# privacy-scaling-explorations/zkevm-specs

Hardware: AMD Instinct MI355X
Metric: BN254 constraint-rows/sec (higher is better)
Workload: dtype u256 (BN254 Fr: 4xu64 canonical cells, u32-limb Montgomery); 1 GPU; EVM circuit, 2^18 execution steps per GPU, mixed-opcode synthetic trace (BASELINE configs[2]); RW table 816377 rows, bytecode table 43913 rows; steps_per_gpu=262144, rw_rows=816377, bytecode_rows=43913, witness_copies=3

## Files before the change

### zkevm_specs_amd/csrc/zkevm_hip.hip

```cpp
#include <hip/hip_runtime.h>
#include <hip/hip_ext.h>
#include <stddef.h>
#include <stdio.h>
#include <string.h>
#include <stdlib.h>
#include <chrono>
#include <string>
#include <vector>

#include <atomic>
#include <mutex>
#include <dlfcn.h>

#include "../../include/zkevm_hip.h"
#include "kernels.hpp"
#include "dist_tally.hpp"
#include "host_index.hpp"
#include "code_dir_build.hpp"

#define ZK_MAX_DEVICES 64
static std::mutex g_dev_mutex;
static hipStream_t g_own_stream[ZK_MAX_DEVICES] = {nullptr};
static hipStream_t g_batch_stream[ZK_MAX_DEVICES][2] = {{nullptr}};
static hipStream_t g_side_stream[ZK_MAX_DEVICES] = {nullptr};
// ... 169 lines not shown
    __shared__ u32 local[EVM_N_BINS];
    if (vblock == 0) {
        if (threadIdx.x == 0 && defer_count) *defer_count = 0u;
        if (threadIdx.x == 0) {
            tally->fail_count = 0ull;
            tally->first_fail = ~0ull;
        }
        for (u32 k = threadIdx.x; k < EVM_N_BINS; k += blockDim.x) taken[k] = 0;
    }
    for (u32 k = threadIdx.x; k < EVM_N_BINS; k += blockDim.x) local[k] = 0;
    __syncthreads();
    u32 i = vblock * blockDim.x + threadIdx.x;
    if (i < n_pairs) {
        const u32 bin = evm_state_bin((u32)steps[((u64)i * STEP_NCELLS + S_STATE) * 4]);
        bin16[i] = (uint16_t)bin;
        atomicAdd(&local[bin], 1u);
    }
    __syncthreads();
    for (u32 k = threadIdx.x; k < EVM_N_BINS; k += blockDim.x)
        if (local[k]) atomicAdd(&hist[k], local[k]);
}
__global__ void evm_state_hist_kernel(const u64* steps, u32 n_pairs, u32* hist, u32* taken, uint16_t* bin16, ZkTally* tally, u32* defer_count) {
    evm_state_hist_body(blockIdx.x, steps, n_pairs, hist, taken, bin16, tally, defer_count);
}
__device__ __forceinline__ void evm_state_scatter_body(u32 vblock, const uint16_t* bin16, u32 n_pairs, const u32* hist, u32* hist_next,
                                                       u32* taken, u32* group_start, u32* perm, u32* early_host = nullptr, u32 early_seq = 0u) {
    __shared__ u32 sa[EVM_N_BINS], sb[EVM_N_BINS];
    __shared__ u32 local[EVM_N_BINS];
    __shared__ u32 base[EVM_N_BINS];
    __shared__ u32 gsh[EVM_N_GROUPS + 1];
    const u32 k = threadIdx.x;
    u32 c = 0, c_real = 0;
    if (k < EVM_N_BINS) {
        c_real = hist[k];
        c = k < (u32)EVM_GROUP_WARM * 128u ? ((c_real + 63u) & ~63u) : c_real;
        sa[k] = c;
        local[k] = 0;
        if (vblock == 0) hist_next[k] = 0;
    }
    __syncthreads();
    u32* src = sa;
    u32* dst = sb;
    for (u32 off = 1; off < EVM_N_BINS; off <<= 1) {
        if (k < EVM_N_BINS) dst[k] = src[k] + (k >= off ? src[k - off] : 0u);
        __syncthreads();
        u32* t = src; src = dst; dst = t;
    }
    u32 excl = 0;
    if (k < EVM_N_BINS) {
        excl = src[k] - c;
        if (vblock == 0) {
            if ((k & 127u) == 0) group_start[k >> 7] = gsh[k >> 7] = excl;
            if (k == EVM_N_BINS - 1) group_start[EVM_N_GROUPS] = gsh[EVM_N_GROUPS] = src[k];
            for (u32 j = c_real; j < c; j++) perm[excl + j] = EVM_NO_PAIR;
        }
    }
    const u32 i = vblock * blockDim.x + threadIdx.x;
    u32 bin = 0, rank = 0;
    if (i < n_pairs) {
        bin = bin16[i];
        rank = atomicAdd(&local[bin], 1u);
    }
    __syncthreads();
    if (vblock == 0 && k == 0 && early_host) {
        __hip_atomic_store(&early_host[EVM_EARLY_WORD], gsh[EVM_GROUP_WARM + 1] - gsh[EVM_GROUP_WARM], __ATOMIC_RELAXED, __HIP_MEMORY_SCOPE_SYSTEM);
        __hip_atomic_store(&early_host[EVM_EARLY_WORD + 1], gsh[EVM_GROUP_COLD + 1] - gsh[EVM_GROUP_COLD], __ATOMIC_RELAXED, __HIP_MEMORY_SCOPE_SYSTEM);
        __threadfence_system();
        __hip_atomic_store(&early_host[EVM_EARLY_WORD + 2], early_seq, __ATOMIC_RELEASE, __HIP_MEMORY_SCOPE_SYSTEM);
    }
    if (k < EVM_N_BINS && local[k]) base[k] = excl + atomicAdd(&taken[k], local[k]);
    __syncthreads();
    if (i < n_pairs) perm[base[bin] + rank] = i;
}
__global__ __launch_bounds__(1024) void evm_state_scatter_kernel(const uint16_t* bin16, u32 n_pairs, const u32* hist, u32* hist_next,
                                                                 u32* taken, u32* group_start, u32* perm) {
    evm_state_scatter_body(blockIdx.x, bin16, n_pairs, hist, hist_next, taken, group_start, perm);
}
__global__ __launch_bounds__(256) void evm_open_fill_kernel(uint4* ff, u64 n_ff, uint4* zero, u64 n_zero) {
    const u64 stride = (u64)gridDim.x * blockDim.x;
    const uint4 F = make_uint4(~0u, ~0u, ~0u, ~0u), Z = make_uint4(0u, 0u, 0u, 0u);
    for (u64 i = (u64)blockIdx.x * blockDim.x + threadIdx.x; i < n_ff; i += stride) ff[i] = F;
    for (u64 i = (u64)blockIdx.x * blockDim.x + threadIdx.x; i < n_zero; i += stride) zero[i] = Z;
}
__device__ __forceinline__ void rw_prepare_quad(const ZkTable& t, u64* keys, EvmDyn* dyn, u32 vthread) {
    const u32 r = vthread >> 2, q = vthread & 3u;
    const bool in = r < t.n;
    uint4 c0 = make_uint4(0, 0, 0, 0), c1 = c0, c2 = c0;
    u64 base = 0;
    u32 flags = 3u;
    if (in) {
        const uint4* p = reinterpret_cast<const uint4*>(t.cells + (u64)r * RW_NCELLS * 4) + q;
        c0 = p[0];
        c1 = p[4];
        c2 = p[8];
        if (q == 0) {
            base = t.cells[0];
            if (t.flags) flags = t.flags[r];
        }
    }
    bool fit, dense_ok;
    u64 w0 = 0, w1 = 0, w2 = 0, w3 = 0;
    const bool z0hi = (c0.y | c0.z | c0.w) == 0u, z1hi = (c1.y | c1.z | c1.w) == 0u, z2hi = (c2.y | c2.z | c2.w) == 0u;
    const bool z0 = z0hi && c0.x == 0u, z1 = z1hi && c1.x == 0u, z2 = z2hi && c2.x == 0u;
    if (q == 0) {
        const u64 rwc = (u64)c0.x | ((u64)c0.y << 32);
        dense_ok = (c0.z | c0.w) == 0u && rwc == base + r && base + r >= base;
        fit = z1hi && c1.x <= 255u;
        w0 = (u64)(c1.x & 0xffu) << 8 | ((u64)(flags & 3u) << 56) | (1ull << 63);
        w2 = (u64)c2.x | ((u64)c2.y << 32);
        w3 = (u64)c2.z | ((u64)c2.w << 32);
    } else if (q == 1) {
        dense_ok = z0;
        fit = z1 && z2hi;
        w0 = (u64)c2.x << 24;
    } else if (q == 2) {
        dense_ok = true;
        fit = z0hi && c0.x <= 255u && (c1.z | c1.w) == 0u && z2hi && c2.x <= 255u;
        w0 = (u64)(c0.x & 0xffu) | ((u64)(c2.x & 0xffu) << 16);
        w1 = (u64)c1.x | ((u64)c1.y << 32);
    } else {
        dense_ok = true;
        fit = z0 && z1 && z2;
    }
    const u32 qshift = threadIdx.x & 60u;
    const bool fits = ((__ballot(fit) >> qshift) & 0xfull) == 0xfull;
    const unsigned long long nd = __ballot(in && !dense_ok);
    if (nd != 0ull && (threadIdx.x & 63u) == 0) atomicOr(&dyn->rw_sparse, 1u);
    if (r == 0 && q == 0 && in) dyn->rw_base = base;
#pragma unroll
    for (int m = 1; m <= 2; m <<= 1) {
        w0 |= __shfl_xor(w0, m);
        w1 |= __shfl_xor(w1, m);
        w2 |= __shfl_xor(w2, m);
        w3 |= __shfl_xor(w3, m);
    }
    if (!fits) w0 = w1 = w2 = w3 = 0;
    if (in && q < 2) {
        const u64 a = q == 0 ? w0 : w2, b2 = q == 0 ? w1 : w3;
        reinterpret_cast<uint4*>(keys + (u64)r * 4)[q] = make_uint4((u32)a, (u32)(a >> 32), (u32)b2, (u32)(b2 >> 32));
    }
}
#define EVM_OPEN_TABLES 8
struct EvmOpenTables {
    ZkTable t[EVM_OPEN_TABLES];
    u32 block_start[EVM_OPEN_TABLES + 2];
    const u64* wds;
    u32 n_wds;
    EvmDyn* dyn;
    ZkTally* tally;
    ZkTable rw;
    u64* rw_keys;
    u32 dir_block0, rw_block0;
    DirBuild dir;
    const u64* steps;
    u32 n_steps;
    u32* step_recs;
    u32 rec_block0;
    EvmSortArgs sort;
    u32 hist_block0;
    u32 lat_period;
#ifdef ZK_DIAG_P1
    u32 diag_skip;
#endif
};
__device__ __forceinline__ void evm_open_small_tables(const EvmOpenTables& o, u32 block) {
    int k = 0;
#pragma unroll
    for (int j = 1; j <= EVM_OPEN_TABLES; j++) k += block >= o.block_start[j] ? 1 : 0;
    const u32 r = (block - o.block_start[k]) * blockDim.x + threadIdx.x;
    if (k == EVM_OPEN_TABLES) {
        const bool nz = r < o.n_wds && !fr_is_zero(fr_load(o.wds + ((u64)r * 4 + 3) * 4));
        const unsigned long long b = __ballot(nz);
        if (b && (threadIdx.x & 63u) == 0) atomicAdd(&o.dyn->agg_total_wds, (u32)__popcll(b));
        return;
    }
    const ZkTable& t = o.t[k];
    const bool in = r < t.n;
    if (k == 0) {
        bool caller = false, present = false, invalid = false, bad = false;
        if (in) {
            const Fr tag = zk_table_cell(t, r, 1), lo = zk_table_cell(t, r, 3), hi = zk_table_cell(t, r, 4);
            caller = fr_eq_u64(tag, 4);
            present = caller && !(fr_is_zero(lo) && fr_is_zero(hi));
            const bool inv_row = fr_eq_u64(tag, 10);
            bad = inv_row && t.flags && (t.flags[r] & 1u);
            invalid = inv_row && fr_eq_u64(lo, 1);
        }
        const unsigned long long bc = __ballot(caller), bp = __ballot(present), bi = __ballot(invalid), bb = __ballot(bad);
        if ((threadIdx.x & 63u) == 0) {
            if (bc) atomicAdd(&o.dyn->agg_max_txs, (u32)__popcll(bc));
            if (bp) atomicAdd(&o.dyn->agg_total_txs, (u32)__popcll(bp));
            if (bi) atomicAdd(&o.dyn->agg_invalid_txs, (u32)__popcll(bi));
            if (bb) atomicOr(&o.dyn->agg_bad_invalid_rows, 1u);
        }
    }
    if (!in) return;
    u64 h;
    switch (k) {
    case 0: h = tx_key_hash(t, r); break;
    case 1: h = blk_key_hash(t, r); break;
    case 2: h = bc_key_hash(t, r); break;
    case 3: h = copy_key_hash(t, r); break;
    case 4: h = keccak_key_hash(t, r); break;
    case 5: h = expt_key_hash(t, r); break;
    case 6: h = sig_key_hash(t, r); break;
    default: h = ecc_key_hash(t, r); break;
    }
    u32* slots = const_cast<u32*>(t.slots);
    u32 s = (u32)h & t.mask;
    while (atomicCAS(&slots[s], ZK_EMPTY_SLOT, r) != ZK_EMPTY_SLOT) s = (s + 1) & t.mask;
}
__global__ __launch_bounds__(256) void evm_open_phase1_kernel(EvmOpenTables o) {
    if (blockIdx.x == 0 && threadIdx.x < 2) {
        o.tally[threadIdx.x].fail_count = 0ull;
        o.tally[threadIdx.x].first_fail = ~0ull;
    }
    u32 b = blockIdx.x;
    if (o.lat_period > 1u && b < o.rec_block0) {
        const u32 q = b / o.lat_period;
        b = (b == q * o.lat_period && q < o.rw_block0) ? q : o.rw_block0 + b - (q + 1u < o.rw_block0 ? q + 1u : o.rw_block0);
    }
#ifdef ZK_DIAG_P1
    {
        const u32 range = b < o.dir_block0 ? 1u : b < o.hist_block0 ? 2u : b < o.rw_block0 ? 4u : b < o.rec_block0 ? 8u : 16u;
        if (o.diag_skip & range) return;
    }
#endif
    if (b < o.dir_block0) evm_open_small_tables(o, b);
    else if (b < o.hist_block0) dirb_events_row(o.dir, (b - o.dir_block0) * blockDim.x + threadIdx.x);
    else if (b < o.rw_block0) evm_state_hist_body(b - o.hist_block0, o.sort.steps, o.sort.n_pairs, o.sort.hist, o.sort.taken, o.sort.bin16, o.sort.tally, o.sort.defer_count);
    else if (b < o.rec_block0) rw_prepare_quad(o.rw, o.rw_keys, o.dyn, (b - o.rw_block0) * blockDim.x + threadIdx.x);
    else evm_step_record_quad(o.steps, o.n_steps, o.step_recs, (b - o.rec_block0) * blockDim.x + threadIdx.x);
}
#define EVM_OPEN_RW_GENERIC_BLOCKS 64u
#define EVM_OPEN_P2_BLOCK 1024u
__global__ __launch_bounds__(1024) void evm_open_phase2_kernel(EvmOpenTables o, u32 scatter_blocks, u32 dir_blocks, u32 force_generic) {
    if (blockIdx.x < scatter_blocks) {
        evm_state_scatter_body(blockIdx.x, o.sort.bin16, o.sort.n_pairs, o.sort.hist, o.sort.hist_next, o.sort.taken, o.sort.group_start, o.sort.perm,
                               o.sort.early_host, o.sort.early_seq);
        return;
    }
    const u32 b = blockIdx.x - scatter_blocks;
    if (b < dir_blocks) {
        dirb_finalize_entry(o.dir, b * blockDim.x + threadIdx.x);
        return;
    }
    if (!force_generic && o.dyn->rw_sparse == 0u) return;
    if (force_generic && b == dir_blocks && threadIdx.x == 0) o.dyn->rw_sparse = 1u;
    u32* slots = const_cast<u32*>(o.rw.slots);
    const u32 stride = (gridDim.x - scatter_blocks - dir_blocks) * blockDim.x;
    for (u32 r = (b - dir_blocks) * blockDim.x + threadIdx.x; r < o.rw.n; r += stride) {
        u32 s = (u32)rw_key_hash(o.rw, r) & o.rw.mask;
        bool dup = false;
        for (;;) {
            const u32 q = atomicCAS(&slots[s], ZK_EMPTY_SLOT, r);
            if (q == ZK_EMPTY_SLOT) break;
            if (!dup && q < o.rw.n) {
                bool same = true;
                for (int c = 0; c < RW_NCELLS && same; c++) same = fr_eq(zk_table_cell(o.rw, q, c), zk_table_cell(o.rw, r, c));
                dup = same;
            }
            s = (s + 1) & o.rw.mask;
        }
        if (dup) atomicAdd(&o.dyn->agg_rw_dups, 1u);
    }
}

__global__ void fr_op_kernel(int op, const u64* a, const u64* b, u64* out, u64 n) {
    u64 i = (u64)blockIdx.x * blockDim.x + threadIdx.x;
    if (i >= n) return;
    Fr x = fr_load(a + 4 * i), y = fr_load(b + 4 * i), r;
    switch (op) {
    case 0: r = fr_add(x, y); break;
    case 1: r = fr_sub(x, y); break;
    case 2: r = fr_mul(x, y); break;
    case 3: r = fr_mont(x, y); break;
    case 4: r = fr_neg(x); break;
    case 5: r = fr_inv(x); break;
    case 6: r = fr_div(x, y); break;
    case 16: r = sp_mul_p(x, y); break;
    case 17: r = sp_sqr_p(x); break;
    case 18: r = ecc_fq_mul_hook(x, y); break;
    case 26: r = sp_sqrt_p(x); break;
    case 27: r = sp_inv_p(x); break;
    default: r = fr_zero();
    }
    for (int k = 0; k < 4; k++) out[4 * i + k] = (u64)r.v[2 * k] | ((u64)r.v[2 * k + 1] << 32);
}

__global__ __launch_bounds__(64) void evm_publish_kernel(const u32* d, u32* h, u32 seq) {
    const u32 i = threadIdx.x;
    if (i < 32u) __hip_atomic_store(&h[i], d[i], __ATOMIC_RELAXED, __HIP_MEMORY_SCOPE_SYSTEM);
    __threadfence_system();
    if (i == 0u) __hip_atomic_store(&h[32], seq, __ATOMIC_RELEASE, __HIP_MEMORY_SCOPE_SYSTEM);
}
struct EvmResultBlock {
    EvmDyn dyn;
    u32 n_deferred_twin;
    u32 pad0[(64 - sizeof(EvmDyn)) / 4 - 1];
    ZkTally tally[2];
    u32 group_start[EVM_N_GROUPS + 1];
    u32 pad1[8 - (EVM_N_GROUPS + 1)];
};
static_assert(sizeof(EvmDyn) <= 64 && sizeof(EvmResultBlock) == 128, "EvmResultBlock layout");
enum SessionKind { SESSION_BCC = 22, SESSION_SGA = 21, SESSION_ECC_ASSIGN = 20, SESSION_ECC = 19, SESSION_PIA = 18, SESSION_EXA = 17, SESSION_TXA = 16, SESSION_WITHDRAWAL = 15, SESSION_REKEY = 14, SESSION_PICOPY = 13, SESSION_PI = 12, SESSION_CPA = 11, SESSION_STATE = 1, SESSION_EVM = 2, SESSION_BYTECODE = 3, SESSION_EXP = 4, SESSION_COPY = 5, SESSION_SIGN = 6, SESSION_KECCAK = 7, SESSION_ASSIGN = 8, SESSION_ECDSA = 9, SESSION_BCA = 10 };

struct zk_session {
    SessionKind kind;
    int device = t_device;
    hipStream_t stream = t_stream;
    u64 n = 0;
    u64 eval_lo = 0, eval_hi = 0;
    bool eval_empty = false;
    std::vector<void*> owned;
    std::vector<int> owned_class;
    ZkTally* d_tally = nullptr;
    u32* d_status = nullptr;
    bool status_external = false;
    std::vector<hipEvent_t> ev;
    u32 launches = 0;
    u32 tally_pass = 0;
    ZkTally* tally_last = nullptr;
    StateArgs state;
    EvmArgs evm;
    BytecodeArgs bytecode;
    ExpArgs exp;
    CopyArgs copy;
    SignArgs sign;
    KeccakGenArgs keccak_gen;
    AssignArgs assign;
    EcdsaArgs ecdsa;
    BcaArgs bca;
    CpaArgs cpa;
// ... 272 lines not shown
    {
        DevArena& A = g_arena[s->device];
        std::lock_guard<std::mutex> lock(A.m);
        for (hipEvent_t e : s->ev) A.events.push_back(e);
        if (s->ev_open0) A.events.push_back(s->ev_open0);
        if (s->ev_open1) A.events.push_back(s->ev_open1);
        if (s->ev_fork) A.events.push_back(s->ev_fork);
        if (s->ev_join) A.events.push_back(s->ev_join);
        if (s->h_result) A.pinned.push_back(s->h_result);
    }
    delete s;
    return 0;
}

extern "C" int zk_state_open(const uint64_t* rows, const uint32_t* flags, uint64_t n, const uint64_t* mpt,
                             uint64_t n_mpt, uint32_t opts, zk_session** out) {
    ARG_TRY(t_device >= 0, "zk_state_open: call zk_init first");
    HIP_TRY(hipSetDevice(t_device));
    ARG_TRY(out && rows && n > 0 && n < (1ull << 32), "zk_state_open: bad arguments");
    ARG_TRY(n_mpt < (1ull << 31), "zk_state_open: MPT table too large");
    const bool dev = opts & ZK_OPT_DEVICE_PTRS;
    const bool compact = opts & ZK_OPT_STATE_COMPACT;
    zk_session* s = new zk_session();
    s->kind = SESSION_STATE;
    s->n = n;
    int rc = 0;
    const void* p = nullptr;
    if ((rc = stage(s, rows, (size_t)n * (compact ? 15 : ST_NCELLS) * 32, dev, &p))) goto fail;
    s->state.rows.cells = (const u64*)p;
    s->state.rows.skip = compact ? 42u : 0u;
    if ((rc = stage(s, flags, (size_t)n * 4, dev, &p))) goto fail;
    s->state.rows.flags = (const u32*)p;
    s->state.rows.n = n;
    s->state.eval_lo = 0;
    s->state.eval_hi = n;
    if ((rc = stage(s, mpt, (size_t)n_mpt * MPT_NCELLS * 32, dev, &p))) goto fail;
    s->state.mpt.cells = (const u64*)p;
    s->state.mpt.flags = nullptr;
    s->state.mpt.n = (u32)n_mpt;
    s->state.mpt.ncells = MPT_NCELLS;
    if ((rc = build_index<state_mpt_key_hash>(s, s->state.mpt, true))) goto fail;
    if ((rc = session_common_init(s))) goto fail;
    *out = s;
    return 0;
fail:
    zk_close(s);
    return rc;
}

static int table_stage(zk_session* s, ZkTable& t, const uint64_t* cells, const uint32_t* flags, uint64_t n,
                       u32 ncells, bool dev) {
    const void* p = nullptr;
    int rc;
    if ((rc = stage(s, cells, (size_t)n * ncells * 32, dev, &p))) return rc;
    t.cells = (const u64*)p;
    if ((rc = stage(s, flags, (size_t)n * 4, dev, &p))) return rc;
    t.flags = (n && flags) ? (const u32*)p : nullptr;
    t.n = (u32)n;
    t.ncells = ncells;
    return 0;
}

#ifndef ZK_HIST_BLOCK
#define ZK_HIST_BLOCK 1024
#endif
static int evm_build_perm(zk_session* s) {
    const u32 n = s->evm.n_pairs;
    u32* h_cur = (s->evm_pass & 1u) ? s->d_hist2 : s->d_hist;
    u32* h_next = (s->evm_pass & 1u) ? s->d_hist : s->d_hist2;
    s->evm_pass++;
    hipLaunchKernelGGL(evm_state_hist_kernel, dim3((n + ZK_HIST_BLOCK - 1) / ZK_HIST_BLOCK), dim3(ZK_HIST_BLOCK), 0, s->stream, s->evm.steps, n, h_cur, s->d_cursor, s->d_bin16, s->d_tally, s->evm.defer_count);
    hipLaunchKernelGGL(evm_state_scatter_kernel, dim3((n + 1023) / 1024), dim3(1024), 0, s->stream, s->d_bin16, n, h_cur, h_next, s->d_cursor,
                       s->d_group_start, s->d_perm);
    HIP_TRY(hipGetLastError());
    return 0;
}

static inline u32 index_cap(u64 n) {
    u32 cap = 16;
    while (cap < 2 * n + 2) cap <<= 1;
    return cap;
}

extern "C" int zk_evm_open(const zk_evm_tables* t, uint32_t opts, zk_session** out) {
    ARG_TRY(t_device >= 0, "zk_evm_open: call zk_init first");
    HIP_TRY(hipSetDevice(t_device));
    ARG_TRY(t && out && t->steps && t->n_steps >= 2 && t->n_steps < (1ull << 32), "zk_evm_open: bad arguments");
    ARG_TRY(t->n_rw < (1ull << 31) && t->n_bytecode < (1ull << 31) && t->n_tx < (1ull << 31) && t->n_block < (1ull << 31) &&
            t->n_copy < (1ull << 31) && t->n_keccak < (1ull << 31) && t->n_exp < (1ull << 31) && t->n_withdrawals < (1ull << 31) &&
            t->n_sig < (1ull << 31) && t->n_ecc < (1ull << 31),
            "zk_evm_open: table too large");
    ARG_TRY(t->aux_cells == 0 || (t->aux_cells >= 2 && t->aux_cells <= 64), "zk_evm_open: aux_cells must be 0 (= 2) or 2..64");
    const bool dev = opts & ZK_OPT_DEVICE_PTRS;
    const bool generic = opts & ZK_OPT_GENERIC_INDEX;
    zk_session* s = new zk_session();
    s->kind = SESSION_EVM;
    s->n = t->n_steps - 1;
    s->side_stream = (opts & ZK_OPT_SIDE_STREAM) != 0;
    int rc = 0;
    const void* p = nullptr;
    EvmArgs& E = s->evm;
    if ((rc = stage(s, t->steps, (size_t)t->n_steps * STEP_NCELLS * 32, dev, &p))) goto fail;
    E.steps = (const u64*)p;
    E.n_steps = t->n_steps;
    E.n_pairs = (u32)(t->n_steps - 1);
    if ((rc = table_stage(s, E.rw, t->rw, t->rw_flags, t->n_rw, RW_NCELLS, dev))) goto fail;
    if ((rc = table_stage(s, E.bytecode, t->bytecode, nullptr, t->n_bytecode, BYTECODE_NCELLS, dev))) goto fail;
    if ((rc = table_stage(s, E.tx, t->tx, t->tx_flags, t->n_tx, TX_NCELLS, dev))) goto fail;
    if ((rc = table_stage(s, E.block, t->block, t->block_flags, t->n_block, BLOCK_NCELLS, dev))) goto fail;
    if ((rc = table_stage(s, E.copy, t->copy, nullptr, t->n_copy, COPY_T_NCELLS, dev))) goto fail;
    if ((rc = table_stage(s, E.keccak, t->keccak, nullptr, t->n_keccak, KECCAK_NCELLS, dev))) goto fail;
    if ((rc = table_stage(s, E.exp, t->exp, nullptr, t->n_exp, EXP_T_NCELLS, dev))) goto fail;
    if ((rc = table_stage(s, E.sig, t->sig, nullptr, t->n_sig, SIG_T_NCELLS, dev))) goto fail;
    if ((rc = table_stage(s, E.ecc, t->ecc, nullptr, t->n_ecc, ECC_T_NCELLS, dev))) goto fail;
    if ((rc = table_stage(s, E.withdrawals, t->withdrawals, nullptr, t->n_withdrawals, 4, dev))) goto fail;
    E.withdrawals.slots = nullptr;
    E.withdrawals.mask = 0;
    E.aux = nullptr;
    E.aux_kind = nullptr;
    E.aux_cells = t->aux_cells ? t->aux_cells : 2u;
    if (t->aux && t->aux_kind) {
        if ((rc = stage(s, t->aux, (size_t)t->n_steps * E.aux_cells * 32, dev, &p))) goto fail;
        E.aux = (const u64*)p;
        if ((rc = stage(s, t->aux_kind, (size_t)t->n_steps * 4, dev, &p))) goto fail;
        E.aux_kind = (const u32*)p;
    }
    {
        ZkTable* const small[EVM_OPEN_TABLES] = {&E.tx, &E.block, &E.bytecode, &E.copy, &E.keccak, &E.exp, &E.sig, &E.ecc};
        const bool want_dir = !generic && t->n_bytecode != 0;
        size_t n_ff = 0;
        u32 caps[EVM_OPEN_TABLES];
        for (int k = 0; k < EVM_OPEN_TABLES; k++) { caps[k] = index_cap(small[k]->n); n_ff += caps[k]; }
        const u32 cap_rw = index_cap(E.rw.n), cap_big = want_dir ? index_cap(t->n_bytecode) : 0u;
        n_ff += (size_t)cap_rw + 2 * (size_t)cap_big + (want_dir ? DIRB_SMALL_SLOTS : 0u);
        u32* ff = nullptr;
        if ((rc = dev_alloc(s, (void**)&ff, n_ff * sizeof(u32)))) goto fail;
        u32* cur = ff;
        for (int k = 0; k < EVM_OPEN_TABLES; k++) { small[k]->slots = cur; small[k]->mask = caps[k] - 1; cur += caps[k]; }
        E.rw.slots = cur; E.rw.mask = cap_rw - 1; cur += cap_rw;
        u32* const dir_rep = cur; cur += cap_big;
        u32* const dir_first = cur; cur += cap_big;
        u32* const small_slots = cur;
        const size_t dyn_bytes = 256, hist_bytes = EVM_N_BINS * sizeof(u32), status_bytes = (((size_t)s->n * sizeof(u32)) + 15) & ~(size_t)15;
        const size_t zero_bytes = dyn_bytes + 2 * hist_bytes + status_bytes + 3 * (size_t)cap_big * 4;
        char* zero = nullptr;
        if ((rc = dev_alloc(s, (void**)&zero, zero_bytes))) goto fail;
        EvmResultBlock* const rb = (EvmResultBlock*)zero;
        EvmDyn* dyn = &rb->dyn;
        s->d_result = rb;
        if ((rc = arena_pinned(s->device, &s->h_result))) goto fail;
        {
            void* hd = nullptr;
            if (hipHostGetDevicePointer(&hd, s->h_result, 0) == hipSuccess) s->h_result_dev = (u32*)hd;
            (void)hipGetLastError();
        }
        static_assert(sizeof(EvmResultBlock) <= 256, "the result block outgrew its slot");
        static_assert((EVM_N_BINS * sizeof(u32)) % 16 == 0, "zero region pieces are 16-byte multiples");
        s->d_hist = (u32*)(zero + dyn_bytes);
        s->d_hist2 = (u32*)(zero + dyn_bytes + hist_bytes);
        s->d_status = (u32*)(zero + dyn_bytes + 2 * hist_bytes);
        u32* const dir_last = (u32*)(zero + dyn_bytes + 2 * hist_bytes + status_bytes);
        E.dyn = dyn;
        E.defer_count = &dyn->n_deferred;
        if ((rc = dev_alloc(s, (void**)&E.defer_list, (size_t)E.n_pairs * sizeof(u32)))) goto fail;
        s->d_tally = rb->tally;
        s->tally_last = s->d_tally;
        {
            const u64 n16 = n_ff / 4 + zero_bytes / 16;
            const u32 fill_grid = (u32)(n16 / 256 < 2048 ? (n16 + 255) / 256 : 2048);
            if (arena_event(s->device, &s->ev_open0) || arena_event(s->device, &s->ev_open1)) s->ev_open0 = s->ev_open1 = nullptr;
            hipExtLaunchKernelGGL(evm_open_fill_kernel, dim3(fill_grid ? fill_grid : 1u), dim3(256), 0, s->stream, s->ev_open0, nullptr, 0, (uint4*)ff,
                                  (u64)(n_ff / 4), (uint4*)zero, (u64)(zero_bytes / 16));
        }
        E.rw_dense = 0;
        E.rw_base = 0;
        E.rw_keys = nullptr;
        E.codes.n = 0;
        E.codes.mask = 0;
        E.codes.packed = nullptr;
        E.codes.entries = nullptr;
        E.codes.slots = nullptr;
        E.agg_max_txs = E.agg_total_txs = E.agg_invalid_txs = E.agg_bad_invalid_rows = E.agg_total_wds = E.agg_rw_dups = 0;
        EvmOpenTables o;
        memset(&o, 0, sizeof o);
        u32 blk = 0;
        for (int k = 0; k < EVM_OPEN_TABLES; k++) { o.t[k] = *small[k]; o.block_start[k] = blk; blk += (small[k]->n + 255u) / 256u; }
        o.block_start[EVM_OPEN_TABLES] = blk;
        blk += (u32)((t->n_withdrawals + 255) / 256);
        o.block_start[EVM_OPEN_TABLES + 1] = blk;
        o.wds = E.withdrawals.cells;
        o.n_wds = (u32)t->n_withdrawals;
        o.dyn = dyn;
        o.tally = s->d_tally;
        o.rw = E.rw;
        if (t->n_rw && !generic) {
            u64* d_keys = nullptr;
            if ((rc = dev_alloc(s, (void**)&d_keys, (size_t)t->n_rw * 32))) goto fail;
            E.rw_keys = d_keys;
            o.rw_keys = d_keys;
        }
        const u32 rw_row_blocks = o.rw_keys ? (u32)((t->n_rw + 63) / 64) : 0u;
        o.dir_block0 = blk;
        u32 dir_row_blocks = 0;
        if (want_dir) {
            DirBuild& d = o.dir;
            d.rows = E.bytecode.cells;
            d.n = (u32)t->n_bytecode;
            d.rep = dir_rep;
            d.first = dir_first;
            d.last = dir_last;
            d.runs = dir_last + cap_big;
            d.bad = dir_last + 2 * (size_t)cap_big;
            d.big_mask = cap_big - 1;
            d.small_slots = small_slots;
            d.dyn = dyn;
            if ((rc = dev_alloc(s, (void**)&d.packed, (size_t)d.n * sizeof(uint16_t)))) goto fail;
            if ((rc = dev_alloc(s, (void**)&d.entries, (size_t)DIRB_MAX_ENTRIES * sizeof(ZkCodeEntry)))) goto fail;
            if ((rc = dev_alloc(s, (void**)&d.list, (size_t)DIRB_MAX_ENTRIES * 4))) goto fail;
            dir_row_blocks = (d.n + 255u) / 256u;
            E.codes.entries = d.entries;
            E.codes.slots = d.small_slots;
            E.codes.packed = d.packed;
        }
        if ((rc = dev_alloc(s, (void**)&s->d_cursor, EVM_N_BINS * sizeof(u32)))) goto fail;
        if ((rc = dev_alloc(s, (void**)&s->d_bin16, (size_t)E.n_pairs * sizeof(uint16_t)))) goto fail;
        s->d_group_start = rb->group_start;
        if ((rc = dev_alloc(s, (void**)&s->d_perm, ((size_t)E.n_pairs + EVM_PERM_PAD + 2 * EVM_HOT_BLOCK) * sizeof(u32)))) goto fail;
        const bool sorted = !(opts & ZK_OPT_NO_STATE_SORT);
        o.hist_block0 = o.dir_block0 + dir_row_blocks;
        u32 hist_blocks = 0, scatter_blocks = 0;
        if (sorted) {
            o.sort.steps = E.steps; o.sort.n_pairs = E.n_pairs; o.sort.hist = s->d_hist; o.sort.hist_next = s->d_hist2;
            o.sort.taken = s->d_cursor; o.sort.bin16 = s->d_bin16; o.sort.group_start = s->d_group_start; o.sort.perm = s->d_perm;
            o.sort.tally = s->d_tally;
            o.sort.defer_count = E.defer_count;
            if ((opts & ZK_OPT_SINGLE_PASS) && s->h_result_dev && evm_lazy_tail_enabled() && !(opts & ZK_OPT_SIDE_STREAM)) {
                static std::atomic<u32> g_early_seq{0};
                u32 q = ++g_early_seq;
                if (!q) q = ++g_early_seq;
                __atomic_store_n(&((u32*)s->h_result)[EVM_EARLY_WORD + 2], 0u, __ATOMIC_RELEASE);
                s->early_seq = q;
                o.sort.early_host = s->h_result_dev;
                o.sort.early_seq = q;
            }
            hist_blocks = (E.n_pairs + 255u) / 256u;
            scatter_blocks = (E.n_pairs + EVM_OPEN_P2_BLOCK - 1u) / EVM_OPEN_P2_BLOCK;
            s->evm_pass = 1;
            s->perm_ready = true;
        }
        o.rw_block0 = o.hist_block0 + hist_blocks;
        o.rec_block0 = o.rw_block0 + rw_row_blocks;
        u32 rec_blocks = 0;
        E.step_recs = nullptr;
        if (!(opts & ZK_OPT_SINGLE_PASS)) {
            u32* recs = nullptr;
            if ((rc = dev_alloc(s, (void**)&recs, (size_t)t->n_steps * EVM_REC_WORDS * sizeof(u32)))) goto fail;
            o.steps = E.steps; o.n_steps = (u32)t->n_steps; o.step_recs = recs;
            E.step_recs = recs;
            rec_blocks = (u32)((t->n_steps + 63) / 64);
        }
        const u32 grid1 = o.rec_block0 + rec_blocks;
        {
            static const u32 spread = [] { const char* e = getenv("ZK_P1_LAT_SPREAD"); const int v = e ? atoi(e) : 2; return (u32)(v < 0 ? 0 : v); }();
            o.lat_period = (o.rw_block0 && spread) ? o.rec_block0 / (spread * o.rw_block0) : 0u;
        }
#ifdef ZK_DIAG_P1
        if (const char* e = getenv("ZK_DIAG_P1_SKIP")) o.diag_skip = (u32)atoi(e);
#endif
        {
            const u32 dir_blocks = want_dir ? DIRB_MAX_ENTRIES / EVM_OPEN_P2_BLOCK : 0u;
            const u32 rw_blocks = t->n_rw ? EVM_OPEN_RW_GENERIC_BLOCKS : 0u;
            bool phase2 = scatter_blocks + dir_blocks + rw_blocks != 0;
#ifdef ZK_DIAG_P1
            if (o.diag_skip) phase2 = false;
#endif
            hipExtLaunchKernelGGL(evm_open_phase1_kernel, dim3(grid1 ? grid1 : 1u), dim3(256), 0, s->stream, nullptr, phase2 ? nullptr : s->ev_open1, 0, o);
            if (phase2)
                hipExtLaunchKernelGGL(evm_open_phase2_kernel, dim3(scatter_blocks + dir_blocks + rw_blocks), dim3(EVM_OPEN_P2_BLOCK), 0, s->stream, nullptr,
                                      s->ev_open1, 0, o, scatter_blocks, dir_blocks, generic ? 1u : 0u);
        }
        if (hipGetLastError() != hipSuccess) { rc = -2; g_err = "zk_evm_open: a build kernel failed to launch"; goto fail; }
    }
    E.opts = (t->begin_with_first_step ? 1u : 0u) | (t->end_with_last_step ? 2u : 0u);
    E.prof = nullptr;
    if (getenv("ZK_EVM_PROF")) {
        if ((rc = dev_alloc(s, (void**)&E.prof, 1024 * 4 * 8 * sizeof(unsigned long long)))) goto fail;
        if (hipMemsetAsync(E.prof, 0, 1024 * 4 * 8 * sizeof(unsigned long long), s->stream) != hipSuccess) { rc = -2; goto fail; }
    }
    E.perm = (opts & ZK_OPT_NO_STATE_SORT) ? nullptr : s->d_perm;
    *out = s;
    return 0;
fail:
    zk_close(s);
    return rc;
}

static void session_timing(zk_session* s, double pass_ms, double* open_ms, double* span_ms);
static int evm_enqueue_tail(zk_session* s);
static bool evm_publish_enqueue(zk_session* s);
extern "C" int zk_evm_verify(const zk_evm_tables* t, uint32_t opts, uint32_t* status_out, zk_result* result) {
    ARG_TRY(result, "zk_evm_verify: result is null");
    zk_session* s = nullptr;
    const auto h0 = std::chrono::steady_clock::now();
    int rc = zk_evm_open(t, opts | ZK_OPT_SINGLE_PASS, &s);
    if (rc) return rc;
    const auto h1 = std::chrono::steady_clock::now();
    const bool dev = opts & ZK_OPT_DEVICE_PTRS;
    rc = zk_launch(s, (dev && status_out) ? status_out : nullptr);
    const auto h2 = std::chrono::steady_clock::now();
    if (!rc) rc = zk_collect(s, result);
    const auto h3 = std::chrono::steady_clock::now();
    if (!rc) {
        t_timing[1] = result->kernel_ms;
        session_timing(s, result->kernel_ms, &t_timing[0], &t_timing[2]);
        for (int k = 0; k < 3; k++) t_timing_sum[k] += t_timing[k];
        t_timing_count++;
    }
    if (!rc && status_out && !dev) rc = zk_read_status(s, status_out);
    zk_close(s);
    const auto h4 = std::chrono::steady_clock::now();
    t_host_phase[0] = std::chrono::duration<double, std::micro>(h1 - h0).count();
    t_host_phase[1] = std::chrono::duration<double, std::micro>(h2 - h1).count();
    t_host_phase[2] = std::chrono::duration<double, std::micro>(h3 - h2).count();
    t_host_phase[3] = std::chrono::duration<double, std::micro>(h4 - h3).count();
    return rc;
}

extern "C" int zk_evm_verify_batch(const zk_evm_tables* const* t, uint64_t n, uint32_t opts, zk_result* results) {
    ARG_TRY(t_device >= 0, "zk_evm_verify_batch: call zk_init first");
    ARG_TRY((t && results) || n == 0, "zk_evm_verify_batch: bad arguments");
    for (uint64_t i = 0; i < n; i++) ARG_TRY(t[i], "zk_evm_verify_batch: null witness");
    HIP_TRY(hipSetDevice(t_device));
    {
        std::lock_guard<std::mutex> lock(g_dev_mutex);
        for (int k = 0; k < 2; k++)
            if (!g_batch_stream[t_device][k]) HIP_TRY(hipStreamCreateWithFlags(&g_batch_stream[t_device][k], hipStreamNonBlocking));
    }
    const hipStream_t caller = t_stream;
    HIP_TRY(hipStreamSynchronize(caller));
    zk_session* pend[2] = {nullptr, nullptr};
    int rc = 0;
    for (uint64_t i = 0; i < n + 2 && !rc; i++) {
        const int slot = (int)(i & 1u);
        if (pend[slot]) {
            rc = zk_collect(pend[slot], &results[i - 2]);
            zk_close(pend[slot]);
            pend[slot] = nullptr;
        }
        if (!rc && i < n) {
            t_stream = g_batch_stream[t_device][slot];
            rc = zk_evm_open(t[i], opts | ZK_OPT_SINGLE_PASS, &pend[slot]);
            t_stream = caller;
            if (!rc) rc = zk_launch(pend[slot], nullptr);
        }
        zk_session* const o = pend[slot ^ 1];
        if (!rc && o && !o->publish_enqueued) {
            rc = evm_enqueue_tail(o);
            if (!rc) o->publish_enqueued = evm_publish_enqueue(o);
        }
    }
    for (int k = 0; k < 2; k++)
        if (pend[k]) zk_close(pend[k]);
    return rc;
}

extern "C" int zk_bytecode_open(const uint64_t* rows, uint64_t n, const uint64_t* keccak, uint64_t n_keccak,
                                const uint64_t* randomness, uint32_t opts, zk_session** out) {
    ARG_TRY(t_device >= 0, "zk_bytecode_open: call zk_init first");
    HIP_TRY(hipSetDevice(t_device));
    ARG_TRY(out && rows && randomness && n > 0 && n < (1ull << 32) && n_keccak < (1ull << 31), "zk_bytecode_open: bad arguments");
    const bool dev = opts & ZK_OPT_DEVICE_PTRS;
    zk_session* s = new zk_session();
    s->kind = SESSION_BYTECODE;
    s->n = n;
    int rc = 0;
    const void* p = nullptr;
    u64 rh[4];
    if ((rc = stage(s, rows, (size_t)n * BC_NCELLS * 32, dev, &p))) goto fail;
    s->bytecode.rows.cells = (const u64*)p;
    s->bytecode.rows.flags = nullptr;
    s->bytecode.rows.n = n;
    if ((rc = table_stage(s, s->bytecode.keccak, keccak, nullptr, n_keccak, KECCAK_NCELLS, dev))) goto fail;
    if ((rc = build_index<keccak_key_hash>(s, s->bytecode.keccak))) goto fail;
    if (dev) {
        if (fetch_small(s->stream, rh, randomness, 32)) { rc = -2; g_err = "randomness download failed"; goto fail; }
    } else {
        memcpy(rh, randomness, 32);
    }
    for (int k = 0; k < 4; k++) { s->bytecode.r.v[2 * k] = (u32)rh[k]; s->bytecode.r.v[2 * k + 1] = (u32)(rh[k] >> 32); }
    {
        u64* d_rm = nullptr;
        if ((rc = dev_alloc(s, (void**)&d_rm, 32))) goto fail;
        zk_launch_fr_to_mont(s->stream, s->bytecode.r, d_rm);
        s->bytecode.r_mont = d_rm;
    }
    if ((rc = session_common_init(s))) goto fail;
    *out = s;
    return 0;
fail:
    zk_close(s);
    return rc;
}

extern "C" int zk_exp_open(const uint64_t* rows, uint64_t n, uint32_t opts, zk_session** out) {
    ARG_TRY(t_device >= 0, "zk_exp_open: call zk_init first");
    HIP_TRY(hipSetDevice(t_device));
    ARG_TRY(out && rows && n > 0 && n < (1ull << 32), "zk_exp_open: bad arguments");
    const bool dev = opts & ZK_OPT_DEVICE_PTRS;
    zk_session* s = new zk_session();
    s->kind = SESSION_EXP;
    s->n = n;
    int rc = 0;
    const void* p = nullptr;
    if ((rc = stage(s, rows, (size_t)n * EX_NCELLS * 32, dev, &p))) goto fail;
    s->exp.rows.cells = (const u64*)p;
    s->exp.rows.flags = nullptr;
    s->exp.rows.n = n;
    if ((rc = session_common_init(s))) goto fail;
    *out = s;
    return 0;
fail:
    zk_close(s);
    return rc;
}

static int build_rw_meta(zk_session* s, const ZkTable& rw, const ZkRwMeta** out) {
    ZkRwMeta* d_meta = nullptr;
    int rc = dev_alloc(s, (void**)&d_meta, sizeof(ZkRwMeta));
    if (rc) return rc;
    static const ZkRwMeta init_dense = {1u, 0u, 0ull}, init_empty = {0u, 0u, 0ull};
    HIP_TRY(hipMemcpyAsync(d_meta, rw.n ? &init_dense : &init_empty, sizeof(ZkRwMeta), hipMemcpyHostToDevice, s->stream));
    if (rw.n) hipLaunchKernelGGL(rw_dense_check_kernel, dim3((rw.n + 255) / 256), dim3(256), 0, s->stream, rw, d_meta);
    *out = d_meta;
    return 0;
// ... 2783 lines not shown
```

Before: 1.592 billion rows/s.

## Move RW key-prepare tail rows into phase-2 kernel and skip unused status buffer

Splits the RW-key preparation so that phase 1 handles only a head fraction of rows (default 5%-tail, set by env var). The remaining tail rows are prepared by extra blocks in the phase-2 kernel, which shortens the critical phase-1 kernel and overlaps that work with the scatter and directory work. Tail rows flag sparsity with a separate bit. If only the tail turns out sparse, the generic path was skipped, so the whole verification is rerun with generic indexing, which is expensive in that case. It also omits allocating and zeroing the status buffer when no status output is requested.

Measured after the change: 1.644 billion rows/s (median of 6 runs). +3.2%, better.

```diff
diff --git a/zkevm_specs_amd/csrc/zkevm_hip.hip b/zkevm_specs_amd/csrc/zkevm_hip.hip
--- a/zkevm_specs_amd/csrc/zkevm_hip.hip
+++ b/zkevm_specs_amd/csrc/zkevm_hip.hip
@@ -275,7 +275,7 @@
     for (u64 i = (u64)blockIdx.x * blockDim.x + threadIdx.x; i < n_ff; i += stride) ff[i] = F;
     for (u64 i = (u64)blockIdx.x * blockDim.x + threadIdx.x; i < n_zero; i += stride) zero[i] = Z;
 }
-__device__ __forceinline__ void rw_prepare_quad(const ZkTable& t, u64* keys, EvmDyn* dyn, u32 vthread) {
+__device__ __forceinline__ void rw_prepare_quad(const ZkTable& t, u64* keys, EvmDyn* dyn, u32 vthread, u32 sparse_bit = 1u) {
     const u32 r = vthread >> 2, q = vthread & 3u;
     const bool in = r < t.n;
     uint4 c0 = make_uint4(0, 0, 0, 0), c1 = c0, c2 = c0;
@@ -318,7 +318,7 @@
     const u32 qshift = threadIdx.x & 60u;
     const bool fits = ((__ballot(fit) >> qshift) & 0xfull) == 0xfull;
     const unsigned long long nd = __ballot(in && !dense_ok);
-    if (nd != 0ull && (threadIdx.x & 63u) == 0) atomicOr(&dyn->rw_sparse, 1u);
+    if (nd != 0ull && (threadIdx.x & 63u) == 0) atomicOr(&dyn->rw_sparse, sparse_bit);
     if (r == 0 && q == 0 && in) dyn->rw_base = base;
 #pragma unroll
     for (int m = 1; m <= 2; m <<= 1) {
@@ -352,6 +352,7 @@
     EvmSortArgs sort;
     u32 hist_block0;
     u32 lat_period;
+    u32 tail_row0, tail_blocks;
 #ifdef ZK_DIAG_P1
     u32 diag_skip;
 #endif
@@ -438,10 +439,15 @@
         dirb_finalize_entry(o.dir, b * blockDim.x + threadIdx.x);
         return;
     }
-    if (!force_generic && o.dyn->rw_sparse == 0u) return;
+    const u32 generic_blocks = gridDim.x - scatter_blocks - dir_blocks - o.tail_blocks;
+    if (b >= dir_blocks + generic_blocks) {
+        rw_prepare_quad(o.rw, o.rw_keys, o.dyn, o.tail_row0 * 4u + (b - dir_blocks - generic_blocks) * blockDim.x + threadIdx.x, 2u);
+        return;
+    }
+    if (!force_generic && (o.dyn->rw_sparse & 1u) == 0u) return;
     if (force_generic && b == dir_blocks && threadIdx.x == 0) o.dyn->rw_sparse = 1u;
     u32* slots = const_cast<u32*>(o.rw.slots);
-    const u32 stride = (gridDim.x - scatter_blocks - dir_blocks) * blockDim.x;
+    const u32 stride = generic_blocks * blockDim.x;
     for (u32 r = (b - dir_blocks) * blockDim.x + threadIdx.x; r < o.rw.n; r += stride) {
         u32 s = (u32)rw_key_hash(o.rw, r) & o.rw.mask;
         bool dup = false;
@@ -880,7 +886,11 @@
     return cap;
 }
 
-extern "C" int zk_evm_open(const zk_evm_tables* t, uint32_t opts, zk_session** out) {
+enum { EVM_OPEN_ONESHOT = 1u, EVM_OPEN_NO_STATUS = 2u };
+#ifndef ZK_P2_RW_TAIL_DEFAULT
+#define ZK_P2_RW_TAIL_DEFAULT 50
+#endif
+static int evm_open_session(const zk_evm_tables* t, uint32_t opts, u32 internal, zk_session** out) {
     ARG_TRY(t_device >= 0, "zk_evm_open: call zk_init first");
     HIP_TRY(hipSetDevice(t_device));
     ARG_TRY(t && out && t->steps && t->n_steps >= 2 && t->n_steps < (1ull << 32), "zk_evm_open: bad arguments");
@@ -939,7 +949,8 @@
         u32* const dir_rep = cur; cur += cap_big;
         u32* const dir_first = cur; cur += cap_big;
         u32* const small_slots = cur;
-        const size_t dyn_bytes = 256, hist_bytes = EVM_N_BINS * sizeof(u32), status_bytes = (((size_t)s->n * sizeof(u32)) + 15) & ~(size_t)15;
+        const bool no_status = (internal & EVM_OPEN_NO_STATUS) != 0;
+        const size_t dyn_bytes = 256, hist_bytes = EVM_N_BINS * sizeof(u32), status_bytes = no_status ? 0 : (((size_t)s->n * sizeof(u32)) + 15) & ~(size_t)15;
         const size_t zero_bytes = dyn_bytes + 2 * hist_bytes + status_bytes + 3 * (size_t)cap_big * 4;
         char* zero = nullptr;
         if ((rc = dev_alloc(s, (void**)&zero, zero_bytes))) goto fail;
@@ -956,7 +967,7 @@
         static_assert((EVM_N_BINS * sizeof(u32)) % 16 == 0, "zero region pieces are 16-byte multiples");
         s->d_hist = (u32*)(zero + dyn_bytes);
         s->d_hist2 = (u32*)(zero + dyn_bytes + hist_bytes);
-        s->d_status = (u32*)(zero + dyn_bytes + 2 * hist_bytes);
+        s->d_status = no_status ? nullptr : (u32*)(zero + dyn_bytes + 2 * hist_bytes);
         u32* const dir_last = (u32*)(zero + dyn_bytes + 2 * hist_bytes + status_bytes);
         E.dyn = dyn;
         E.defer_count = &dyn->n_deferred;
@@ -997,7 +1008,17 @@
             E.rw_keys = d_keys;
             o.rw_keys = d_keys;
         }
-        const u32 rw_row_blocks = o.rw_keys ? (u32)((t->n_rw + 63) / 64) : 0u;
+        u64 n_head = t->n_rw;
+        if ((internal & EVM_OPEN_ONESHOT) && o.rw_keys && t->n_rw < (1ull << 30)) {
+            static const u32 tail_pm = [] { const char* e = getenv("ZK_P2_RW_TAIL"); const int v = e ? atoi(e) : ZK_P2_RW_TAIL_DEFAULT; return (u32)(v < 0 ? 0 : v > 999 ? 999 : v); }();
+            const u64 h = (t->n_rw - t->n_rw * tail_pm / 1000 + 63) & ~63ull;
+            if (h < t->n_rw) n_head = h;
+        }
+        const u32 rw_row_blocks = o.rw_keys ? (u32)((n_head + 63) / 64) : 0u;
+        if (n_head < t->n_rw) {
+            o.tail_row0 = (u32)n_head;
+            o.tail_blocks = (u32)((t->n_rw - n_head + EVM_OPEN_P2_BLOCK / 4 - 1) / (EVM_OPEN_P2_BLOCK / 4));
+        }
         o.dir_block0 = blk;
         u32 dir_row_blocks = 0;
         if (want_dir) {
@@ -1061,6 +1082,7 @@
         {
             static const u32 spread = [] { const char* e = getenv("ZK_P1_LAT_SPREAD"); const int v = e ? atoi(e) : 2; return (u32)(v < 0 ? 0 : v); }();
             o.lat_period = (o.rw_block0 && spread) ? o.rec_block0 / (spread * o.rw_block0) : 0u;
+            if (o.tail_blocks && o.lat_period > 1u) o.lat_period |= 1u;
         }
 #ifdef ZK_DIAG_P1
         if (const char* e = getenv("ZK_DIAG_P1_SKIP")) o.diag_skip = (u32)atoi(e);
@@ -1068,13 +1090,13 @@
         {
             const u32 dir_blocks = want_dir ? DIRB_MAX_ENTRIES / EVM_OPEN_P2_BLOCK : 0u;
             const u32 rw_blocks = t->n_rw ? EVM_OPEN_RW_GENERIC_BLOCKS : 0u;
-            bool phase2 = scatter_blocks + dir_blocks + rw_blocks != 0;
+            bool phase2 = scatter_blocks + dir_blocks + rw_blocks + o.tail_blocks != 0;
 #ifdef ZK_DIAG_P1
             if (o.diag_skip) phase2 = false;
 #endif
             hipExtLaunchKernelGGL(evm_open_phase1_kernel, dim3(grid1 ? grid1 : 1u), dim3(256), 0, s->stream, nullptr, phase2 ? nullptr : s->ev_open1, 0, o);
             if (phase2)
-                hipExtLaunchKernelGGL(evm_open_phase2_kernel, dim3(scatter_blocks + dir_blocks + rw_blocks), dim3(EVM_OPEN_P2_BLOCK), 0, s->stream, nullptr,
+                hipExtLaunchKernelGGL(evm_open_phase2_kernel, dim3(scatter_blocks + dir_blocks + rw_blocks + o.tail_blocks), dim3(EVM_OPEN_P2_BLOCK), 0, s->stream, nullptr,
                                       s->ev_open1, 0, o, scatter_blocks, dir_blocks, generic ? 1u : 0u);
         }
         if (hipGetLastError() != hipSuccess) { rc = -2; g_err = "zk_evm_open: a build kernel failed to launch"; goto fail; }
@@ -1092,15 +1114,20 @@
     zk_close(s);
     return rc;
 }
+extern "C" int zk_evm_open(const zk_evm_tables* t, uint32_t opts, zk_session** out) { return evm_open_session(t, opts, 0u, out); }
+
+static bool evm_sparse_tail_only(const zk_session* s) {
+    return s->kind == SESSION_EVM && s->h_result && ((const EvmResultBlock*)s->h_result)->dyn.rw_sparse == 2u;
+}
 
 static void session_timing(zk_session* s, double pass_ms, double* open_ms, double* span_ms);
 static int evm_enqueue_tail(zk_session* s);
 static bool evm_publish_enqueue(zk_session* s);
-extern "C" int zk_evm_verify(const zk_evm_tables* t, uint32_t opts, uint32_t* status_out, zk_result* result) {
-    ARG_TRY(result, "zk_evm_verify: result is null");
+static int evm_oneshot_run(const zk_evm_tables* t, uint32_t opts, uint32_t* status_out, zk_result* result, bool* redo, double host_us[4]) {
     zk_session* s = nullptr;
+    *redo = false;
     const auto h0 = std::chrono::steady_clock::now();
-    int rc = zk_evm_open(t, opts | ZK_OPT_SINGLE_PASS, &s);
+    int rc = evm_open_session(t, opts | ZK_OPT_SINGLE_PASS, EVM_OPEN_ONESHOT | (status_out ? 0u : EVM_OPEN_NO_STATUS), &s);
     if (rc) return rc;
     const auto h1 = std::chrono::steady_clock::now();
     const bool dev = opts & ZK_OPT_DEVICE_PTRS;
@@ -1108,19 +1135,34 @@
     const auto h2 = std::chrono::steady_clock::now();
     if (!rc) rc = zk_collect(s, result);
     const auto h3 = std::chrono::steady_clock::now();
-    if (!rc) {
+    if (!rc) *redo = evm_sparse_tail_only(s);
+    if (!rc && !*redo) {
         t_timing[1] = result->kernel_ms;
         session_timing(s, result->kernel_ms, &t_timing[0], &t_timing[2]);
         for (int k = 0; k < 3; k++) t_timing_sum[k] += t_timing[k];
         t_timing_count++;
     }
-    if (!rc && status_out && !dev) rc = zk_read_status(s, status_out);
+    if (!rc && !*redo && status_out && !dev) rc = zk_read_status(s, status_out);
     zk_close(s);
     const auto h4 = std::chrono::steady_clock::now();
-    t_host_phase[0] = std::chrono::duration<double, std::micro>(h1 - h0).count();
-    t_host_phase[1] = std::chrono::duration<double, std::micro>(h2 - h1).count();
-    t_host_phase[2] = std::chrono::duration<double, std::micro>(h3 - h2).count();
-    t_host_phase[3] = std::chrono::duration<double, std::micro>(h4 - h3).count();
+    host_us[0] = std::chrono::duration<double, std::micro>(h1 - h0).count();
+    host_us[1] = std::chrono::duration<double, std::micro>(h2 - h1).count();
+    host_us[2] = std::chrono::duration<double, std::micro>(h3 - h2).count();
+    host_us[3] = std::chrono::duration<double, std::micro>(h4 - h3).count();
+    return rc;
+}
+extern "C" int zk_evm_verify(const zk_evm_tables* t, uint32_t opts, uint32_t* status_out, zk_result* result) {
+    ARG_TRY(result, "zk_evm_verify: result is null");
+    bool redo = false;
+    double us[4] = {0, 0, 0, 0};
+    int rc = evm_oneshot_run(t, opts, status_out, result, &redo, us);
+    if (!rc && redo) {
+        const double first = us[0] + us[1] + us[2] + us[3];
+        rc = evm_oneshot_run(t, opts | ZK_OPT_GENERIC_INDEX, status_out, result, &redo, us);
+        us[0] += first;
+    }
+    if (rc && us[0] == 0) return rc;
+    for (int k = 0; k < 4; k++) t_host_phase[k] = us[k];
     return rc;
 }
 
@@ -1142,12 +1184,22 @@
         const int slot = (int)(i & 1u);
         if (pend[slot]) {
             rc = zk_collect(pend[slot], &results[i - 2]);
+            const bool redo = !rc && evm_sparse_tail_only(pend[slot]);
             zk_close(pend[slot]);
             pend[slot] = nullptr;
+            if (redo) {
+                t_stream = g_batch_stream[t_device][slot];
+                rc = evm_open_session(t[i - 2], opts | ZK_OPT_SINGLE_PASS | ZK_OPT_GENERIC_INDEX, EVM_OPEN_ONESHOT | EVM_OPEN_NO_STATUS, &pend[slot]);
+                t_stream = caller;
+                if (!rc) rc = zk_launch(pend[slot], nullptr);
+                if (!rc) rc = zk_collect(pend[slot], &results[i - 2]);
+                if (pend[slot]) zk_close(pend[slot]);
+                pend[slot] = nullptr;
+            }
         }
         if (!rc && i < n) {
             t_stream = g_batch_stream[t_device][slot];
-            rc = zk_evm_open(t[i], opts | ZK_OPT_SINGLE_PASS, &pend[slot]);
+            rc = evm_open_session(t[i], opts | ZK_OPT_SINGLE_PASS, EVM_OPEN_ONESHOT | EVM_OPEN_NO_STATUS, &pend[slot]);
             t_stream = caller;
             if (!rc) rc = zk_launch(pend[slot], nullptr);
         }
```
